# ducha-aiki/mods

Measured on AMD Instinct MI355X. Metric: image-pairs/sec (1024x768, HessAff+RootSIFT over the affine view ladder, MFMA FGINN match, LO-RANSAC H), higher is better.
Workload: dtype f32 (detect/describe) + u8 on the int8 matrix cores (distance matrix)

## Files before the change

include/modsx.h:

```cpp
#ifndef MODSX_H
#define MODSX_H
#include <stdint.h>
#ifdef __cplusplus
extern "C" {
#endif

#define MODSX_VERSION 100

typedef enum modsx_status {
  MODSX_OK = 0,
  MODSX_ERR_ARG = -1,
  MODSX_ERR_DEVICE = -2,
  MODSX_ERR_NOMEM = -3,
  MODSX_ERR_INTERNAL = -4,
  MODSX_ERR_CAPACITY = -5,
  MODSX_ERR_TIMEOUT = -6
} modsx_status;

enum { MODSX_FIXED_TH = 0, MODSX_RELATIVE_TH = 1, MODSX_FIXED_REG_NUMBER = 2, MODSX_RELATIVE_REG_NUMBER = 3,
       MODSX_NOT_LESS_THAN_REGIONS = 4 };
enum { MODSX_DET_HESSIAN = 0, MODSX_DET_DOG = 1, MODSX_DET_HARRIS = 2, MODSX_DET_MSER = 3 };
enum { MODSX_DESC_SIFT = 0, MODSX_DESC_ROOT_SIFT = 1, MODSX_DESC_HALF_SIFT = 2, MODSX_DESC_HALF_ROOT_SIFT = 3 };
#define MODSX_MAX_DESC 4
enum { MODSX_HESSIAN_DARK = 0, MODSX_HESSIAN_BRIGHT = 1, MODSX_HESSIAN_SADDLE = 2 };
// ... 166 lines not shown
int modsx_loransac_f(const double *pts, const double *laf1, const double *laf2, int T, double err_threshold,
                     double confidence, int max_samples, int localOptimization, double LAFCoef, int doSymmCheck,
                     int error_type, unsigned seed, double *F, unsigned char *inl, unsigned char *keep, int *data_out);
int modsx_verify_device_stats(long *out, int reset);
int modsx_verify_device_timing(long *out, int reset);

int modsx_match_pair(modsx_ctx *ctx, const modsx_image *img1, const modsx_image *img2,
                     const modsx_pair_params *par, modsx_pair_result *res);
void modsx_pair_result_release(modsx_pair_result *res);

int modsx_match_pairs(modsx_ctx *const *ctxs, int n_ctx, const modsx_image *const *imgs1,
                      const modsx_image *const *imgs2, int n_pairs, const modsx_pair_params *par,
                      modsx_pair_result *results);

int modsx_match_pairs_views(modsx_ctx *const *ctxs, int n_ctx, const modsx_image *const *imgs1,
                            const modsx_image *const *imgs2, int n_pairs, const modsx_view *views, int n_views,
                            const modsx_pair_params *par, modsx_pair_result *results);

int modsx_last_batch_verify(double *sum_ms, int *pairs, int *threads);
int modsx_last_match_geometry(int *qs, int *fat, int *S, int *tiles_per_split, int *ntiles_ub);
int modsx_debug_orientation_counts(unsigned long long *launched, unsigned long long *skipped, int reset);
int modsx_debug_reproject_certain_drop(const modsx_region *regs, int n, const double *H, int orig_w, int orig_h, double boxk,
                                       unsigned char *drop);
int modsx_last_timings(modsx_ctx *ctx, double *ms6);

int modsx_set_vs_pars(const double *scale_set, int ns, const double *tilt_set, int nt, double phi_base,
                      double InitSigma, int doBlur, modsx_view *par, int cap, modsx_view *prev, int *nprev,
                      int cap_prev);

modsx_image *modsx_synth_view(modsx_ctx *ctx, const modsx_image *gray, const modsx_view *view, double *H9,
                              int *is_identity);

int modsx_detect_describe_views(modsx_ctx *ctx, const modsx_image *img, const modsx_view *views, int nviews,
                                const modsx_pair_params *par, int view_begin, int view_step, modsx_region **regs,
                                float **desc, void *dev_desc_u8, long dev_cap, int *view_counts);

int modsx_match_fginn_device(modsx_ctx *ctx, const void *dev_desc1_u8, int n1, const void *dev_desc2_u8, int n2,
                             const double *pos2, double ratio, double contradDist, int nn, modsx_tentative **out);

#define MODSX_DB_MAX_ROWS 16777216L
typedef struct modsx_db modsx_db;
modsx_db *modsx_db_create(modsx_ctx *ctx, const void *rows, long n, int dtype);
void modsx_db_free(modsx_ctx *ctx, modsx_db *db);
long modsx_db_rows(const modsx_db *db);
int modsx_db_nearest(modsx_ctx *ctx, const modsx_db *db, const float *desc, int n, float *dmin);
int modsx_match_fginn_db(modsx_ctx *ctx, const float *desc1, int n1, const float *desc2, int n2, const double *pos2,
// ... 102 lines not shown
```

mods_amd/__init__.py:

```python
import ctypes as C
import os
import subprocess

import numpy as np

_HERE = os.path.dirname(os.path.abspath(__file__))
LIB_PATH = os.environ.get("MODSX_LIB", os.path.join(_HERE, "libmodsx.so"))

KEYPOINT = np.dtype([("x", "f8"), ("y", "f8"), ("a11", "f8"), ("a12", "f8"), ("a21", "f8"), ("a22", "f8"),
                     ("s", "f8"), ("response", "f8"), ("octave_number", "i4"), ("pyramid_scale", "f8"),
                     ("sub_type", "i4")], align=True)
REGION = np.dtype([("img_id", "i4"), ("img_reproj_id", "i4"), ("id", "i4"), ("parent_id", "i4"), ("type", "i4"),
                   ("det_kp", KEYPOINT), ("reproj_kp", KEYPOINT)], align=True)
SSKP = np.dtype([("octave", "i4"), ("level", "i4"), ("r0", "i4"), ("c0", "i4"), ("r", "i4"), ("c", "i4"),
                 ("type", "i4"), ("pad", "i4"), ("b0", "f4"), ("b1", "f4"), ("b2", "f4"), ("val", "f4"),
                 ("x", "f4"), ("y", "f4"), ("s", "f4"), ("pixelDistance", "f4")], align=True)
TENT = np.dtype([("q", "i4"), ("t0", "i4"), ("tj", "i4"), ("t1", "i4"), ("d1", "f8"), ("d2", "f8"),
                 ("d2by2ndcl", "f8"), ("ratio", "f8")], align=True)


class HessAffParams(C.Structure):
    _fields_ = [("threshold", C.c_float), ("mode", C.c_int), ("reg_number", C.c_int),
                ("rel_threshold", C.c_float), ("rel_reg_number", C.c_float), ("numberOfScales", C.c_int),
                ("initialSigma", C.c_float), ("edgeEigenValueRatio", C.c_double), ("border", C.c_int),
# ... 52 lines not shown


class RepClassSel(C.Structure):
    _fields_ = [("detector", C.c_int), ("desc_type", C.c_int), ("ratio", C.c_double)]


EXPORTS = ["modsx_version", "modsx_last_error", "modsx_free", "modsx_create", "modsx_destroy", "modsx_synchronize",
           "modsx_default_hessaff_params", "modsx_default_pair_params", "modsx_image_upload", "modsx_image_update",
           "modsx_image_wrap_device", "modsx_image_free", "modsx_image_download", "modsx_detect_affine_keypoints",
           "modsx_detect_scalespace", "modsx_octave_levels", "modsx_gaussian_blur", "modsx_resize_half", "modsx_response",
           "modsx_detect_affine_regions", "modsx_detect_orientation", "modsx_reproject_regions", "modsx_reproject_regions_touch_boundary",
           "modsx_describe_regions", "modsx_match_fginn", "modsx_duplicate_filtering", "modsx_ransac_h",
           "modsx_loransac_h", "modsx_ransac_h_errtype", "modsx_loransac_h_errtype", "modsx_ransac_f", "modsx_loransac_f", "modsx_match_pair", "modsx_match_pairs", "modsx_match_pairs_views", "modsx_pair_result_release",
           "modsx_set_vs_pars", "modsx_synth_view", "modsx_detect_describe_views", "modsx_match_fginn_device",
           "modsx_match_pair_views", "modsx_match_ladder", "modsx_save_regions", "modsx_load_regions", "modsx_default_mser_params", "modsx_detect_msers", "modsx_detect_msers_u8", "modsx_last_timings", "modsx_profile",
           "modsx_kernel_stats", "modsx_last_batch_verify", "modsx_last_match_geometry", "modsx_comm_unique_id", "modsx_comm_create", "modsx_comm_destroy", "modsx_comm_info",
           "modsx_view_block_order", "modsx_detect_describe_views_sharded", "modsx_match_fginn_sharded",
           "modsx_match_pair_views_sharded", "modsx_match_pairs_views_sharded", "modsx_match_ladder_sharded", "modsx_comm_loopback_id", "modsx_comm_set_lanes",
           "modsx_comm_attach", "modsx_comm_lane_done", "modsx_comm_reset_lanes", "modsx_comm_set_timeout", "modsx_comm_stats",
           "modsx_shard_block_bytes", "modsx_shard_block_pack", "modsx_shard_blocks_unpack", "modsx_shard_device_pack",
           "modsx_shard_device_unpack", "modsx_verify_device_stats", "modsx_verify_device_timing", "modsx_comm_set_exchange",
           "modsx_shard_owner_plan", "modsx_db_create", "modsx_db_free", "modsx_db_rows", "modsx_db_nearest",
           "modsx_match_fginn_db", "modsx_match_fginn_db_device", "modsx_set_fginn_db",
           "modsx_debug_orientation_counts", "modsx_debug_reproject_certain_drop",
           "modsx_rep_create", "modsx_rep_free", "modsx_rep_add_views", "modsx_rep_append", "modsx_rep_class",
           "modsx_rep_match_fginn", "modsx_match_reps", "modsx_match_one_to_many"]
EXPORTS_DEGENSAC = ["exp_ransacHcustom", "exp_ransacFcustom", "HDs", "HDsi", "HDsidx", "HDsSym", "HDsiSym", "HDsSymidx",
                    "HDsSymMax", "HDsiSymMax", "HDsSymidxMax", "FDs", "FDsSym", "exFDs", "exFDsSym",
                    "modsx_ransac_set_seed"]

SHARD_ROW_REGION, SHARD_ROW_KP = 0, 1
EXCHANGE_ALL_GATHER, EXCHANGE_OWNER = 0, 1
KP_FIELDS = ("x", "y", "a11", "a12", "a21", "a22", "s")
KERNEL_CLASSES = ["blur_hess", "hessian", "resize", "nms_localize", "baumberg", "orientation", "patch_sample",
                  "blur_rows", "describe", "match_fginn", "gray", "warp_affine", "view_blur", "blur_cols", "match_sweep1", "match_db"]


def build(force=False):
    src = os.path.join(_HERE, "csrc")
    srcs = [os.path.join(src, f) for f in os.listdir(src) if f.endswith((".hip", ".cpp", ".hpp"))]
    srcs.append(os.path.join(_HERE, "..", "include", "modsx.h"))
    stale = (not os.path.exists(LIB_PATH)) or any(os.path.getmtime(s) > os.path.getmtime(LIB_PATH) for s in srcs)
    if force or stale:
        subprocess.check_call(["make", "-C", src, "-j8"], stdout=subprocess.DEVNULL)
    return LIB_PATH


# ... 19 lines not shown
        L.modsx_comm_lane_done.argtypes = [C.c_void_p, C.c_int]
        L.modsx_comm_reset_lanes.argtypes = [C.c_void_p]
        L.modsx_comm_set_timeout.argtypes = [C.c_void_p, C.c_int]
        L.modsx_comm_stats.argtypes = [C.c_void_p, C.c_void_p, C.c_int]
        L.modsx_destroy.argtypes = [C.c_void_p]
        L.modsx_free.argtypes = [C.c_void_p]
        L.modsx_image_upload.restype = C.c_void_p
        L.modsx_image_upload.argtypes = [C.c_void_p, C.c_void_p, C.c_int, C.c_int, C.c_int, C.c_int]
        L.modsx_image_update.argtypes = [C.c_void_p, C.c_void_p, C.c_void_p, C.c_int, C.c_int, C.c_int, C.c_int]
        L.modsx_debug_last_batch_verify_each.argtypes = [C.c_void_p, C.c_int]
        L.modsx_image_wrap_device.restype = C.c_void_p
        L.modsx_image_wrap_device.argtypes = [C.c_void_p, C.c_void_p, C.c_int, C.c_int]
        L.modsx_image_free.argtypes = [C.c_void_p, C.c_void_p]
        L.modsx_db_create.restype = C.c_void_p
        L.modsx_db_create.argtypes = [C.c_void_p, C.c_void_p, C.c_long, C.c_int]
        L.modsx_db_free.restype = None
        L.modsx_db_free.argtypes = [C.c_void_p, C.c_void_p]
        L.modsx_db_rows.restype = C.c_long
        L.modsx_db_rows.argtypes = [C.c_void_p]
        L.modsx_db_nearest.argtypes = [C.c_void_p, C.c_void_p, C.c_void_p, C.c_int, C.c_void_p]
        L.modsx_set_fginn_db.argtypes = [C.c_void_p, C.c_void_p]
        L.modsx_debug_reproject_certain_drop.argtypes = [C.c_void_p, C.c_int, C.c_void_p, C.c_int, C.c_int, C.c_double, C.c_void_p]
        L.modsx_debug_orientation_counts.argtypes = [C.c_void_p, C.c_void_p, C.c_int]
        L.modsx_rep_create.restype = C.c_void_p
        L.modsx_rep_create.argtypes = [C.c_void_p]
        L.modsx_rep_free.restype = None
        L.modsx_rep_free.argtypes = [C.c_void_p, C.c_void_p]
        L.modsx_rep_add_views.argtypes = [C.c_void_p, C.c_void_p, C.c_void_p, C.c_void_p, C.c_void_p]
        L.modsx_rep_append.argtypes = [C.c_void_p, C.c_void_p, C.c_int, C.c_int, C.c_void_p, C.c_void_p, C.c_int, C.c_int]
        L.modsx_rep_class.argtypes = [C.c_void_p, C.c_void_p, C.c_int, C.c_int, C.c_void_p, C.c_void_p]
        L.modsx_rep_match_fginn.argtypes = [C.c_void_p, C.c_void_p, C.c_void_p, C.c_int, C.c_int, C.c_double, C.c_double, C.c_int,
                                            C.c_void_p]
        L.modsx_match_reps.argtypes = [C.c_void_p, C.c_int, C.c_void_p, C.c_void_p, C.c_int, C.c_void_p, C.c_int, C.c_void_p,
                                       C.c_void_p]
        L.modsx_match_one_to_many.argtypes = [C.c_void_p, C.c_int, C.c_void_p, C.c_void_p, C.c_int, C.c_void_p, C.c_int, C.c_int,
                                              C.c_void_p, C.c_void_p, C.c_void_p]
        L.modsx_synth_view.restype = C.c_void_p
        L.modsx_synth_view.argtypes = [C.c_void_p, C.c_void_p, C.c_void_p, C.c_void_p, C.c_void_p]
        _lib = L
    return _lib


def _err():
    return lib().modsx_last_error().decode()


# ... 616 lines not shown
    out = np.zeros(max(n, 1), np.float64)
    n = min(n, lib().modsx_debug_last_batch_verify_each(_p(out), len(out)))
    return out[:n]


def last_batch_verify():
    ms, n, t = C.c_double(), C.c_int(), C.c_int()
    lib().modsx_last_batch_verify(C.byref(ms), C.byref(n), C.byref(t))
    return ms.value, n.value, t.value


def last_match_geometry():
    v = [C.c_int() for _ in range(5)]
    lib().modsx_last_match_geometry(*[C.byref(x) for x in v])
    return dict(zip(("qs", "fat", "S", "tiles_per_split", "ntiles_ub"), (x.value for x in v)))


def orientation_counts(reset=False):
    a, b = C.c_ulonglong(), C.c_ulonglong()
    lib().modsx_debug_orientation_counts(C.byref(a), C.byref(b), int(reset))
    return a.value, b.value


def reproject_certain_drop(regs, H, w, h, boxk=2 * 3.0 * 3.0 ** 0.5):
    regs = np.ascontiguousarray(regs, REGION)
    H = np.ascontiguousarray(H, np.float64).reshape(9)
    drop = np.zeros(max(1, len(regs)), np.uint8)
    _check(lib().modsx_debug_reproject_certain_drop(_p(regs), len(regs), _p(H), int(w), int(h), C.c_double(boxk), _p(drop)),
           "reproject_certain_drop")
    return drop[:len(regs)].astype(bool)


def view_block_order(counts):
    counts = np.ascontiguousarray(counts, np.int32)
    world, nviews = counts.shape
    total = int(counts.sum())
    src = np.zeros(max(1, total), np.int32)
    mr = C.c_int(0)
    n = _check(lib().modsx_view_block_order(_p(counts), world, nviews, _p(src), len(src), C.byref(mr)), "view_block_order")
    return src[:n].copy(), mr.value


def shard_owner_plan(item_counts, nviews, world, rank, image_owner):
    cnt = np.ascontiguousarray(item_counts, np.int32)
    own = np.ascontiguousarray(image_owner, np.int32)
    nimg = len(own)
# ... 151 lines not shown
```

mods_amd/csrc/capi.hip:

```cpp
#include <math.h>
#include <malloc.h>
#include <atomic>
#include <chrono>
#include <mutex>
#include <thread>
#include <condition_variable>
#include <deque>
#include "engine_api.hpp"

using namespace mx;

#define NEED(c)                                             \
  do {                                                      \
    if (!(c)) { mx::set_error("null argument: " #c); return MODSX_ERR_ARG; } \
  } while (0)

template <typename T>
static T *to_malloc(const std::vector<T> &v) {
  T *p = (T *)malloc(sizeof(T) * (v.size() ? v.size() : 1));
  if (p && !v.empty()) memcpy(p, v.data(), sizeof(T) * v.size());
  return p;
}

static std::atomic<long> g_verifyUs(0);
// ... 303 lines not shown
  *out = to_malloc(vout[0]);
  return (int)vout[0].size();
}

int modsx_reproject_regions(modsx_region *regs, int n, const double *H, int orig_w, int orig_h) {
  if (n < 0 || (n > 0 && !regs) || !H) { mx::set_error("modsx_reproject_regions: bad argument"); return MODSX_ERR_ARG; }
  return reproject_regions(regs, n, H, orig_w, orig_h);
}

int modsx_reproject_regions_touch_boundary(modsx_region *regs, int n, const double *H, int orig_w, int orig_h, double mrSize) {
  if (n < 0 || (n > 0 && !regs) || !H) { mx::set_error("modsx_reproject_regions_touch_boundary: bad argument"); return MODSX_ERR_ARG; }
  return reproject_regions_box(regs, n, H, orig_w, orig_h, mrSize);
}

int modsx_debug_reproject_certain_drop(const modsx_region *regs, int n, const double *H, int orig_w, int orig_h, double boxk,
                                       unsigned char *drop) {
  if (n < 0 || (n > 0 && (!regs || !drop)) || !H) { mx::set_error("modsx_debug_reproject_certain_drop: bad argument"); return MODSX_ERR_ARG; }
  reproject_certain_drop(regs, n, H, orig_w, orig_h, boxk, drop);
  return n;
}

int modsx_debug_orientation_counts(unsigned long long *launched, unsigned long long *skipped, int reset) {
  mx::orientation_counts(launched, skipped, reset != 0);
  return MODSX_OK;
}

int modsx_describe_regions(modsx_ctx *ctx, const modsx_image *img, const modsx_region *regs, int n, double mrSize,
                           int patchSize, int fast_extraction, int photoNorm, int desc_type, double maxBinValue,
                           float *desc) {
  NEED(ctx); NEED(img);
  if (n < 0 || (n > 0 && (!regs || !desc))) { mx::set_error("modsx_describe_regions: bad argument"); return MODSX_ERR_ARG; }
  if (desc_type < MODSX_DESC_SIFT || desc_type > MODSX_DESC_HALF_ROOT_SIFT) { mx::set_error("descriptor type"); return MODSX_ERR_ARG; }
  hipSetDevice(ctx->dev);
  std::vector<modsx_region> v[1];
  v[0].assign(regs, regs + n);
  const modsx_image *imgs[1] = {img};
  float *hosts[1] = {desc};
  int rc = describe_batch(ctx, imgs, 1, v, mrSize, patchSize, fast_extraction, photoNorm, desc_type, maxBinValue, hosts,
                          nullptr, nullptr);
  if (rc) return rc;
  return n;
}

int modsx_match_fginn(modsx_ctx *ctx, const float *desc1, int n1, const float *desc2, int n2, const double *pos2,
                      double ratio, double contradDist, int nn, modsx_tentative **out) {
  NEED(ctx); NEED(out);
// ... 748 lines not shown
```

mods_amd/csrc/engine.hip:

```cpp
#include <atomic>
#include <math.h>
#include <stdio.h>
#include <algorithm>
#include <chrono>
#include <map>
#include <unordered_set>
#include <mutex>
#include <string>
#include "engine_api.hpp"

#ifdef MODSX_DUP_BUILD
namespace mx {
int dup_count(int cls) {
  static const long mask = getenv("MODSX_DUP") ? strtol(getenv("MODSX_DUP"), nullptr, 0) : 0;
  return 1 + (int)((mask >> cls) & 1);
}
}
#endif
namespace mx {

static thread_local std::string g_err;
void set_error(const std::string &s) { g_err = s; }
static std::atomic<int> g_busyContexts{0};
bool gpu_shared() { return g_busyContexts.load(std::memory_order_relaxed) > 1; }
// ... 175 lines not shown
  Profiler &p = c->prof;
  p.enabled = enable; p.used = 0;
  for (int i = 0; i < K_NCLASS; i++) { p.ms[i] = 0; p.work[i] = 0; p.launches[i] = 0; }
}

static int upload_tables(modsx_ctx *c) {
  const int PS = 41;
  std::vector<float> m(PS * PS);
  circular_gauss_mask(m.data(), PS, PS / 3.0f);
  {
    const int PSP = 44;
    std::vector<unsigned short> idx;
    std::vector<float> w;
    for (int r = 1; r < PS - 1; r++)
      for (int q = 1; q < PS - 1; q++)
        if (m[r * PS + q] > 0) { idx.push_back((unsigned short)(r * PSP + q)); w.push_back(m[r * PS + q]); }
    for (int r = 0; r < PS; r++)
      for (int q = 0; q < PS; q++)
        if ((r == 0 || q == 0 || r == PS - 1 || q == PS - 1) && m[r * PS + q] > 0) {
          set_error("orientation mask reaches the patch frame");
          return MODSX_ERR_ARG;
        }
    if ((int)idx.size() > ORI_NV) { set_error("orientation voting list exceeds ORI_NV"); return MODSX_ERR_ARG; }
    while ((int)idx.size() < ORI_NV) { idx.push_back((unsigned short)(PSP + 1)); w.push_back(0.f); }
    {
      constexpr int PER_L = ORI_NV / 64;
      std::vector<unsigned short> idx2(ORI_NV);
      std::vector<float> w2(ORI_NV);
      for (int l = 0; l < 64; l++)
        for (int q = 0; q < PER_L; q++) { idx2[l + 64 * q] = idx[PER_L * l + q]; w2[l + 64 * q] = w[PER_L * l + q]; }
      idx.swap(idx2); w.swap(w2);
    }
    MX_HIP(hipMalloc(&c->dOriMask, ORI_NV * 4));
    MX_HIP(hipMalloc(&c->dOriIdx, ORI_NV * 2));
    MX_HIP(hipMemcpy(c->dOriMask, w.data(), ORI_NV * 4, hipMemcpyHostToDevice));
    MX_HIP(hipMemcpy(c->dOriIdx, idx.data(), ORI_NV * 2, hipMemcpyHostToDevice));
  }
  MX_HIP(hipMalloc(&c->dSiftMask, PS * PS * 4));
  circular_gauss_mask(m.data(), PS, 0);
  MX_HIP(hipMemcpy(c->dSiftMask, m.data(), PS * PS * 4, hipMemcpyHostToDevice));
  {
    std::vector<unsigned short> idx;
    for (int i = 0; i < PS * PS; i++) if (m[i] > 0) idx.push_back((unsigned short)i);
    c->nSiftMask = (int)idx.size();
    MX_HIP(hipMalloc(&c->dSiftMaskIdx, idx.size() * 2));
    MX_HIP(hipMemcpy(c->dSiftMaskIdx, idx.data(), idx.size() * 2, hipMemcpyHostToDevice));
  }
  MX_HIP(hipMalloc(&c->dAtan, 256 * 8));
  MX_HIP(hipMemcpy(c->dAtan, atan_lut_host(), 256 * 8, hipMemcpyHostToDevice));
  {
    std::vector<unsigned char> obin(ATAN_CASES);
    std::vector<float> so(ATAN_CASES);
    const double *L = atan_lut_host();
    const float PIf = float(M_PI);
    const double TWO_PI = 6.28318530718;
    for (int e = 0; e < ATAN_CASES; e++) {
      const float ori = e < 2048 ? atan2lut_value(L, e >> 8, e & 255) : 0.f;
      obin[e] = (unsigned char)(int)(36 * (ori / PIf + 1.0f) / 2.0f);
      so[e] = (float)((double)8.0f * ((double)ori + TWO_PI) / TWO_PI);
// ... 60 lines not shown
  for (int i = 0; i < 6; i++) c->timings[i] = 0;
  if (upload_tables(c) != MODSX_OK) { delete c; return nullptr; }
  return c;
}

void ctx_destroy(modsx_ctx *c) {
  if (!c) return;
  ctx_worker_stop(c);
  if (c->peer) { ctx_destroy(c->peer); c->peer = nullptr; }
  if (c->half) { ctx_destroy(c->half); c->half = nullptr; }
  hipSetDevice(c->dev);
  hipStreamSynchronize(c->stream);
  for (int i = 0; i < MAXB; i++) c->pyr[i].store.release();
  DevBuf *bufs[] = {&c->nmsJobs, &c->cand, &c->counter, &c->affJobs, &c->affOut, &c->oriJobs, &c->oriOut, &c->descJobs, &c->tilePrefix,
                    &c->taps, &c->imgRefs, &c->scratchA, &c->scratchB, &c->descAllF[0], &c->descAllF[1], &c->descAllU8[0],
                    &c->descAllU8[1], &c->descAllU8b[0], &c->descAllU8b[1], &c->shardLocal, &c->pos2, &c->matchRows, &c->matchWork, &c->dbSel, &c->misc, &c->scratchC, &c->needTab, &c->coordTab, &c->tileJob, &c->blurTiles, &c->nmsQueue, &c->rowStarts, &c->viewTmp[0], &c->viewTmp[1], &c->viewTaps, &c->viewJobs};
  for (DevBuf *b : bufs) b->release();
  for (int i = 0; i < MAXB; i++) { c->descF[i].release(); c->descU8[i].release(); c->viewImg[i].release(); for (int k = 0; k < 3; k++) c->descU8x[k][i].release(); }
  for (int d = 0; d < 2; d++) for (int t = 0; t < 4; t++) for (int sd = 0; sd < 2; sd++) c->descCls[d][t][sd].release();
  for (int t = 0; t < 4; t++) c->halfDesc[t].release();
  c->candSort.release(); c->candOut.release();
  PinBuf *pins[] = {&c->hCand, &c->hAff, &c->hOri, &c->hDesc, &c->hMisc, &c->hNms, &c->hMatch, &c->hViewTaps, &c->hViewJobs, &c->hMser};
  for (PinBuf *b : pins) b->release();
  hipFree(c->dSmmMask); hipFree(c->dOriMask); hipFree(c->dOriIdx); hipFree(c->dSiftMask); hipFree(c->dSiftMaskIdx); hipFree(c->dAtan); hipFree(c->dOriBinTab); hipFree(c->dSiftOTab); hipFree(c->dSiftBins);
  hipFree(c->dSiftW);
  for (int i = 0; i < 2; i++) hipEventDestroy(c->descEv[i]);
  c->hDescB.release(); c->hRefs.release();
  hipStreamDestroy(c->stream);
  if (c->hFlag) hipHostFree(c->hFlag);
  delete c;
}

static const double K_SIGMA = 2 * 3.0 * sqrt(3.0);

void desc_class_order(const DescSet &ds, int *ord) {
  int m = 0;
  for (int type = 3; type >= 0; type--)
    for (int i = 0; i < ds.n; i++) if (ds.type[i] == type) ord[m++] = i;
}
int resolve_descs(const modsx_pair_params &pp, const modsx_ladder_step *st, DescSet &ds) {
  const int ns = st ? st->n_desc : 0;
  if (ns < 0 || ns > MODSX_MAX_DESC || pp.n_desc < 0 || pp.n_desc > MODSX_MAX_DESC) { set_error("n_desc must be 0..4"); return MODSX_ERR_ARG; }
  if (ns > 0) { ds.n = ns; for (int i = 0; i < ns; i++) { ds.type[i] = st->desc_types[i]; ds.ratio[i] = st->desc_ratios[i]; } }
  else if (pp.n_desc > 0) { ds.n = pp.n_desc; for (int i = 0; i < ds.n; i++) { ds.type[i] = pp.desc_types[i]; ds.ratio[i] = pp.desc_ratios[i]; } }
  else { ds.n = 1; ds.type[0] = pp.desc_type; ds.ratio[0] = st && st->match_ratio > 0 ? st->match_ratio : pp.match_ratio; }
  for (int i = 0; i < ds.n; i++) {
    if (ds.type[i] < 0 || ds.type[i] > 3) { set_error("descriptor type must be 0..3 (SIFT, RootSIFT, HalfSIFT, HalfRootSIFT)"); return MODSX_ERR_ARG; }
// ... 3 lines not shown
}

static int upload_img_refs(modsx_ctx *c, const modsx_image *const *imgs, int n) {
  const bool fresh = !c->imgRefs.p;
  if (!c->imgRefs.ensure(MAXB * sizeof(ImgRef))) return MODSX_ERR_NOMEM;
  ImgRef refs[MAXB];
  memset(refs, 0, sizeof refs);
  for (int i = 0; i < n; i++) { refs[i].d = imgs[i]->d; refs[i].rows = imgs[i]->rows; refs[i].cols = imgs[i]->cols; }
  if (!fresh && memcmp(refs, c->imgRefsHost, sizeof refs) == 0) return MODSX_OK;
  if (!c->hRefs.ensure(sizeof refs)) return MODSX_ERR_NOMEM;
  memcpy(c->hRefs.p, refs, sizeof refs);
  MX_HIP(ctx_copy(c, c->imgRefs.p, c->hRefs.p, sizeof refs, hipMemcpyHostToDevice));
  memcpy(c->imgRefsHost, refs, sizeof refs);
  return MODSX_OK;
}

static double eye_test(const double *H) {
  return fabs(H[0] - 1.0) + fabs(H[1]) + fabs(H[2]) + fabs(H[3]) + fabs(H[4] - 1.0) + fabs(H[5]) + fabs(H[6]) + fabs(H[7]) +
         fabs(H[8] - 1.0);
}
static bool is_eye(const double *H) { return eye_test(H) < 0.01; }
static bool ori_prefilter_on() {
  static const bool on = !(getenv("MODSX_ORI_PREFILTER") && atoi(getenv("MODSX_ORI_PREFILTER")) == 0);
  return on;
}
static std::atomic<unsigned long long> g_oriLaunched{0}, g_oriSkipped{0};
void orientation_counts(unsigned long long *launched, unsigned long long *skipped, bool reset) {
  if (launched) *launched = reset ? g_oriLaunched.exchange(0) : g_oriLaunched.load();
  else if (reset) g_oriLaunched.store(0);
  if (skipped) *skipped = reset ? g_oriSkipped.exchange(0) : g_oriSkipped.load();
  else if (reset) g_oriSkipped.store(0);
}

int detect_orientation_batch(modsx_ctx *c, const modsx_image *const *imgs, int n, const std::vector<modsx_region> *in,
                             double mrSize, int patchSize, int doHalfSIFT, int maxAngNum, double th, int addUpRight,
                             std::vector<modsx_region> *out, const OriReproj *reproj) {
  if (patchSize != 41) { set_error("orientation patchSize must be 41"); return MODSX_ERR_ARG; }
  const bool prefilter = reproj && ori_prefilter_on();
  for (int i = 0; i < n; i++) out[i].clear();
  double mrScale = (double)mrSize;
  int patchImageSize = 2 * int(mrScale) + 1;
  double imageToPatchScale = double(patchImageSize) / (double)patchSize;
  HostMark hm;
  std::vector<OriJob> jobs;
  std::vector<char> passed[MAXB];
  std::vector<unsigned char> certain[MAXB];
// ... 30 lines not shown
  jobStart[0] = 0;
  for (int i = 0; i < n; i++) jobStart[i + 1] = jobStart[i] + jobsOf[i].size();
  jobs.resize(jobStart[n]);
  g_oriLaunched.fetch_add(jobStart[n], std::memory_order_relaxed);
  host_parallel_light(n, [&](int i) { if (!jobsOf[i].empty()) memcpy(jobs.data() + jobStart[i], jobsOf[i].data(), jobsOf[i].size() * sizeof(OriJob)); });
  hm.mark("orientation jobs");
  const float *res = nullptr;
  const int maxA = maxAngNum < 0 ? ORI_MAX_PEAKS : std::min(maxAngNum, ORI_MAX_PEAKS);
  const size_t oriB = (size_t)(1 + maxA) * 4;
  if (!jobs.empty()) {
    int rc = upload_img_refs(c, imgs, n);
    if (rc) return rc;
    hipStream_t s = c->stream;
    size_t nj = jobs.size();
    if (!c->oriJobs.ensure(nj * sizeof(OriJob)) || !c->oriOut.ensure(nj * oriB) ||
        !c->hOri.ensure(nj * (sizeof(OriJob) + oriB)))
      return MODSX_ERR_NOMEM;
    memcpy(c->hOri.p, jobs.data(), nj * sizeof(OriJob));
    float *hres = (float *)((char *)c->hOri.p + nj * sizeof(OriJob));
    res = hres;
    MX_HIP(ctx_copy(c, c->oriJobs.p, c->hOri.p, nj * sizeof(OriJob), hipMemcpyHostToDevice));
    ProfScope ps(c, K_ORIENT, (double)nj * 41 * 41 * 4);
    launch_orientation(s, (OriJob *)c->oriJobs.p, (float *)c->oriOut.p, (int)nj, (ImgRef *)c->imgRefs.p, c->dOriIdx,
                       c->dOriMask, c->dOriBinTab, doHalfSIFT, th, maxA);
    MX_HIP(ctx_copy(c, hres, c->oriOut.p, nj * oriB, hipMemcpyDeviceToHost));
    MX_HIP(ctx_sync(c));
  }
  hm.mark("orientation launch + wait");
  host_parallel_light(n, [&](int i) {
    size_t jk = jobStart[i];
    out[i].clear();
    out[i].reserve(in[i].size() + in[i].size() / 4);
    for (size_t r = 0; r < in[i].size(); r++) {
      if (!passed[i][r]) continue;
      const modsx_region &base = in[i][r];
      if (maxAngNum > 0) {
        const float *o = res + (jk++) * (size_t)(1 + maxA);
        int on;
        memcpy(&on, o, 4);
        const double b11 = base.det_kp.a11, b12 = base.det_kp.a12, b21 = base.det_kp.a21, b22 = base.det_kp.a22;
        for (int a = 0; a < on; a++) {
          double ci = cosf(-o[1 + a]);
          double si = sinf(-o[1 + a]);
          out[i].push_back(base);
          modsx_region &t = out[i].back();
          t.id = 0;
          t.det_kp.a11 = b11 * ci - b12 * si;
// ... 809 lines not shown
```

mods_amd/csrc/engine.hpp:

```cpp
#pragma once
#include <hip/hip_runtime.h>
#include <stdint.h>
#include <stdlib.h>
#include <string.h>
#include <string>
#include <vector>
#include "../../include/modsx.h"
#include "kmath.hpp"

namespace mx {

#ifndef MODSX_MAXB
#define MODSX_MAXB 32
#endif
constexpr int MAXB = MODSX_MAXB;
constexpr int PAIR_GROUP = 4;
constexpr int NMS_MAXJ = 1024;
constexpr int MAX_TAPS = 17;

struct BlurJob {
  const float *src;
  float *blur;
  float *resp;
  int rows, cols;
// ... 153 lines not shown
inline bool check_borders_host(int w, int h, float ofsx, float ofsy, float a11, float a12, float a21, float a22, int rw, int rh) {
  return check_borders(w, h, ofsx, ofsy, a11, a12, a21, a22, rw, rh);
}
bool invert3(const double *S, double *t);
void rectify(double &a11, double &a12, double &a21, double &a22);

void launch_blur_hess(hipStream_t s, const BlurBatch &b, int nj, int maxRows, int maxCols);
void launch_hessian(hipStream_t s, const BlurBatch &b, int nj, int maxRows, int maxCols);
void launch_resize_half(hipStream_t s, const ResizeBatch &b, int nj, int maxRows, int maxCols);
void launch_nms(hipStream_t s, const NmsBatch &b, const NmsJob *jobs, const int *tilePrefix, const int *tileJob, int nj,
                int nTiles, int4 *queue, unsigned *qcount, unsigned qcap, Candidate *out, unsigned *counter, unsigned cap,
                const int *octFirst = nullptr, int levelsPerOctave = 0);
size_t cand_sort_temp_bytes(unsigned nsort);
int launch_cand_order(hipStream_t s, const Candidate *cand, const unsigned *counter, unsigned nsort, unsigned long long *keys,
                      unsigned long long *keys2, unsigned *idx, unsigned *idx2, void *temp, size_t tempBytes, unsigned long long *tabKey,
                      unsigned *tabRank, unsigned tabSize, unsigned *slotOf, Candidate *out, unsigned *outCount);
constexpr int NMS_QUEUES = 64;
constexpr int NMS_TILE_ROWS = 16;
void launch_gray(hipStream_t s, const void *src, float *dst, size_t n, int channels, int dtype);
void launch_baumberg(hipStream_t s, const AffJob *jobs, AffOut *out, int n, const float *mask, int W, int maxIter,
                     float convTh, float affInitialSigma);
constexpr int ATAN_CASES = 2048 + 64;
constexpr int ORI_NV = 1344;
void launch_orientation(hipStream_t s, const OriJob *jobs, float *out, int n, const ImgRef *imgs,
                        const unsigned short *maskIdx, const float *maskW,
                        const unsigned char *binTab, int doHalf, double th, int maxAngles);
void launch_trunc_u8(hipStream_t s, const float *src, uint8_t *dst, size_t n);
size_t mser_sort_blocks(const int *rows, int n);
void launch_mser_sort(hipStream_t s, const uint8_t *const *u8, const int *rows, const int *cols, const size_t *ordOfs, int n, int *blockHist,
                      int *start, int *order);
void launch_expand_blur_tiles(hipStream_t s, const DescJob *jobs, const int *prefixRows, const int *prefixCols, int nJobs,
                              const int *needTab, BlurTile *tilesRows, BlurTile *tilesCols, float2 *rowStarts);
void launch_sample_rows(hipStream_t s, const DescJob *jobs, const BlurTile *tiles, int nTiles, const ImgRef *imgs, const float *taps,
                        const int *needTab, float *dst, const float2 *rowStarts, float *dstGrid);
void launch_blur_cols(hipStream_t s, const BlurTile *tiles, int nTiles, const float *taps, const int *needTab, const float *src,
                      float *dst);
void launch_expand_tiles(hipStream_t s, const int *prefix, int nJobs, int *tileJob);
void launch_patch_sample(hipStream_t s, const DescJob *jobs, const int *tilePrefix, const int *tileJob, int nTiles,
                         const ImgRef *imgs, float *scratch);
void launch_patch_blur(hipStream_t s, const DescJob *jobs, const int *tilePrefix, const int *tileJob, int nTiles,
                       const float *taps, const int *needTab, const float *src, float *dst, int pass);
void launch_describe(hipStream_t s, const DescJob *jobs, int n, const ImgRef *imgs, const float *grid,
                     const int *needTab, const float *coordTab,
                     const float *mask, const unsigned short *maskIdx, int nmask, const float *oTab, const int *bins,
                     const double *wts, int photoNorm, int descTypes, int nOut, double maxBin, const DescOut &outs);
void launch_warp_affine(hipStream_t s, const WarpJob &jb);
void launch_blur_pass(hipStream_t s, const float *src, float *dst, int rows, int cols, const float *taps, int n, int pass, int border = 0);
void launch_sub(hipStream_t s, const float *a, const float *b, float *o, size_t n);
// ... 83 lines not shown
  size_t lastSurvivors = 0;
  mx::DevBuf nmsJobs, cand, counter, affJobs, affOut, oriJobs, oriOut, descJobs, tilePrefix, taps, imgRefs, scratchA, scratchB,
      descF[mx::MAXB], descU8[mx::MAXB], descAllF[2], descAllU8[2], descAllU8b[2], descCls[2][4][2], descU8x[3][mx::MAXB], shardLocal, pos2, matchRows, matchWork, dbSel, misc, viewTmp[2], viewTaps, viewJobs, viewImg[mx::MAXB], scratchC, needTab, coordTab, tileJob, blurTiles, nmsQueue, rowStarts;
  mx::ImgRef imgRefsHost[mx::MAXB];
  mx::PinBuf hDescB;
  hipEvent_t descEv[2];
  bool descEvPending[2] = {false, false};
  bool descByEvent[2] = {true, true};
  unsigned descMark[2] = {0, 0};
  unsigned *hFlag = nullptr;
  unsigned flagSeq = 0;
  bool waitRuntime = true;
  mx::PinBuf hCand, hAff, hOri, hDesc, hMisc, hNms, hMatch, hViewTaps, hViewJobs, hMser, hRefs;
  float *dSmmMask = nullptr;
  int smmW = 0;
  std::vector<uint64_t> candKeys, candKeys2, candClaim;
  std::vector<uint32_t> candOrder, candOrder2;
  float *dOriMask = nullptr;
  unsigned short *dOriIdx = nullptr;
  float *dSiftMask = nullptr;
  unsigned short *dSiftMaskIdx = nullptr;
  int nSiftMask = 0;
  double *dAtan = nullptr;
  unsigned char *dOriBinTab = nullptr;
  float *dSiftOTab = nullptr;
  int *dSiftBins = nullptr;
  double *dSiftW = nullptr;
  double timings[6];
  mx::Profiler prof;
  size_t lastCandCount = 0;
  const mx::DbSet *fginnDb = nullptr;
  int busyDepth = 0;
  int shardLane = 0;
  modsx_ctx *peer = nullptr;
  modsx_ctx *half = nullptr;
  mx::DevBuf halfDesc[4];
  void *worker = nullptr;
};
```

mods_amd/csrc/kernels_orient.hip:

```cpp
#include "engine.hpp"

namespace mx {

constexpr int PS = 41, PSP = 44;
constexpr int ORI_B = 21;

template <bool LDS_TABLE>
__global__ __launch_bounds__(64) void k_orientation(const OriJob *jobs, float *out, int n, const ImgRef *imgs,
                                                    const unsigned short *maskIdx, const float *maskW,
                                                    const unsigned char *binTab, int doHalf, double th, int maxAngles) {
  const int k = xcd_chunk(blockIdx.x, n);
  if (k >= n) return;
  const int lane = threadIdx.x;
  __shared__ __attribute__((aligned(16))) float bufX[PS * PSP];
  __shared__ __attribute__((aligned(16))) unsigned char sbtLds[LDS_TABLE ? ATAN_CASES : 16];
  const unsigned char *const sbt = LDS_TABLE ? sbtLds : binTab;
  __shared__ float hist[40];
  static_assert(ATAN_CASES == 33 * 64, "one 4-byte word per lane and step");
  if (LDS_TABLE) {
    unsigned t[9];
#pragma unroll
    for (int u = 0; u < 9; u++) t[u] = lane + 64 * u < ATAN_CASES / 4 ? reinterpret_cast<const unsigned *>(binTab)[lane + 64 * u] : 0u;
#pragma unroll
    for (int u = 0; u < 9; u++)
      if (lane + 64 * u < ATAN_CASES / 4) reinterpret_cast<unsigned *>(sbtLds)[lane + 64 * u] = t[u];
  }
  const OriJob jb = jobs[k];
  const ImgRef im = imgs[jb.img];
  const int half = PS >> 1;
  const bool touch = check_borders(im.cols, im.rows, jb.x, jb.y, jb.a11, jb.a12, jb.a21, jb.a22, PS, PS);
  {
    float rx = jb.x - (float)half * jb.a12, ry = jb.y - (float)half * jb.a22;
#pragma unroll
    for (int j = 1; j < PS; j++)
      if (lane >= j) { rx += jb.a12; ry += jb.a22; }
    if (lane < PS) {
      float WX = rx - (float)half * jb.a11;
      float WY = ry - (float)half * jb.a21;
      float *row = bufX + lane * PSP;
      for (int i0 = 0; i0 < PS; i0 += ORI_B) {
        float t[ORI_B];
        if (!touch) {
#pragma unroll
          for (int u = 0; u < ORI_B; u++) {
            t[u] = i0 + u < PS ? bilinear_tap(as_global(im.d), im.rows, im.cols, WX, WY, false) : 0.f;
            WX += jb.a11; WY += jb.a21;
          }
        } else {
#pragma unroll
          for (int u = 0; u < ORI_B; u++) {
            t[u] = i0 + u < PS ? bilinear_tap(as_global(im.d), im.rows, im.cols, WX, WY, true) : 0.f;
            WX += jb.a11; WY += jb.a21;
          }
        }
#pragma unroll
        for (int u = 0; u < ORI_B; u++)
          if (i0 + u < PS) row[i0 + u] = t[u];
      }
    }
  }
  __syncthreads();
  const float PIf = float(M_PI);
  constexpr int PER_L = ORI_NV / 64;
  float wreg[PER_L];
  unsigned char breg[PER_L];
#pragma unroll
  for (int q = 0; q < PER_L; q++) {
    const int e = lane + 64 * q;
    const int p = maskIdx[e];
    const float m = maskW[e];
    const float xg = bufX[p + 1] - bufX[p - 1];
    const float yg = bufX[p + PSP] - bufX[p - PSP];
    const float mag = sqrtf(xg * xg + yg * yg);
    int code, idx;
    const bool special = atan2lut_case(yg, xg, code, idx);
    unsigned char bin = 255;
    float w = 0.f;
    if (m > 0 && mag > 1.0f) {
      bin = sbt[special ? 2048 : code * 256 + idx];
      w = mag * m;
// ... 84 lines not shown
  float mx = lane < nb ? hv : 0.f;
#pragma unroll
  for (int off = 32; off > 0; off >>= 1) mx = fmaxf(mx, __shfl_xor(mx, off));
  const float thresh = (float)((double)(mx > 0.f ? mx : 0.f) * th);
  if (doHalf) {
    const float other = __shfl(hv, lane < nb / 2 ? lane + nb / 2 : lane);
    if (lane < nb / 2) hv += other;
    else if (lane < nb) hv = 0.f;
  }
  const float ha = __shfl(hv, lane == 0 ? nb - 1 : lane - 1);
  const float hc = __shfl(hv, lane == nb - 1 ? 0 : lane + 1);
  const bool peak = lane < nb && hv >= thresh && hv > ha && hv > hc;
  const unsigned long long peaks = __ballot(peak);
  const int rank = __popcll(peaks & ((1ull << lane) - 1ull));
  float *const o = out + (size_t)k * (1 + maxAngles);
  if (lane == 0) o[0] = __int_as_float(min(__popcll(peaks), maxAngles));
  if (peak && rank < maxAngles) {
    const float pp = (ha - hc) / (ha - 2.0f * hv + hc) / 2.0f;
    o[1 + rank] = 2.0f * PIf * ((float)lane + 0.5f + pp) / (float)nb - PIf;
  }
}

void launch_orientation(hipStream_t s, const OriJob *jobs, float *out, int n, const ImgRef *imgs,
                          const unsigned short *maskIdx, const float *maskW, const unsigned char *binTab, int doHalf, double th,
                          int maxAngles) {
  if (n <= 0) return;
  if (n < 2 * 256 * 16)
    MX_DUP(K_ORIENT) hipLaunchKernelGGL(k_orientation<true>, dim3(8 * ((n + 7) / 8)), dim3(64), 0, s, jobs, out, n, imgs, maskIdx, maskW, binTab, doHalf, th,
                       maxAngles);
  else
    MX_DUP(K_ORIENT) hipLaunchKernelGGL(k_orientation<false>, dim3(8 * ((n + 7) / 8)), dim3(64), 0, s, jobs, out, n, imgs, maskIdx, maskW, binTab, doHalf, th,
                       maxAngles);
}

}
```

mods_amd/csrc/tables.cpp:

```cpp
#include <math.h>
#include <stdio.h>
#include "engine.hpp"

namespace mx {

std::vector<float> gaussian_kernel(int n, double sigma) {
  std::vector<float> k(n);
  double sigmaX = sigma > 0 ? sigma : ((n - 1) * 0.5 - 1) * 0.3 + 0.8;
  double scale2X = -0.5 / (sigmaX * sigmaX);
  double sum = 0;
  for (int i = 0; i < n; i++) {
    double x = i - (n - 1) * 0.5;
    double t = exp(scale2X * x * x);
    k[i] = (float)t;
    sum += k[i];
  }
  sum = 1. / sum;
  for (int i = 0; i < n; i++) k[i] = (float)(k[i] * sum);
  return k;
}

int blur_ksize(float sigma) {
  int size = (int)(2.0 * 3.0 * sigma + 1.0);
  if (size % 2 == 0) size++;
// ... 9 lines not shown
  int endSize = int(ceilf(scale * 5.0f) - halfSize);
  for (int i = 1; i < endSize; i++) tmp[halfSize - i] += expf(float((i + halfSize) * (i + halfSize)) / scale2);
  for (int i = 0; i <= halfSize; i++)
    for (int j = 0; j <= halfSize; j++) {
      float v = tmp[i] * tmp[j];
      mask[(i + halfSize) * size + (-j + halfSize)] = v;
      mask[(-i + halfSize) * size + (j + halfSize)] = v;
      mask[(i + halfSize) * size + (j + halfSize)] = v;
      mask[(-i + halfSize) * size + (-j + halfSize)] = v;
    }
}

void circular_gauss_mask(float *mask, int size, float sigma) {
  int halfSize = size >> 1;
  float r2 = float(halfSize * halfSize);
  float sigma2 = (sigma == 0) ? 0.9f * r2 : 2 * sigma * sigma;
  for (int i = 0; i < size; i++)
    for (int j = 0; j < size; j++) {
      float disq = float((i - halfSize) * (i - halfSize) + (j - halfSize) * (j - halfSize));
      mask[i * size + j] = (disq < r2) ? expf(-disq / sigma2) : 0;
    }
}

const double *atan_lut_host() {
  static double lut[256];
  static bool ready = false;
  if (!ready) {
    for (int i = 0; i < 256; i++) {
      char buf[64];
      snprintf(buf, sizeof buf, "%.10f", atan(i / 255.0));
      lut[i] = strtod(buf, nullptr);
    }
    lut[32] = 0.1248376255;
    lut[83] = 0.3146752558;
    lut[100] = 0.3737268255;
    ready = true;
  }
  return lut;
}

bool invert3(const double *S, double *t) {
  double d = S[0] * (S[4] * S[8] - S[5] * S[7]) - S[1] * (S[3] * S[8] - S[5] * S[6]) + S[2] * (S[3] * S[7] - S[4] * S[6]);
  if (d == 0.) { for (int i = 0; i < 9; i++) t[i] = 0; return false; }
  d = 1. / d;
  t[0] = (S[4] * S[8] - S[5] * S[7]) * d; t[1] = (S[2] * S[7] - S[1] * S[8]) * d; t[2] = (S[1] * S[5] - S[2] * S[4]) * d;
  t[3] = (S[5] * S[6] - S[3] * S[8]) * d; t[4] = (S[0] * S[8] - S[2] * S[6]) * d; t[5] = (S[2] * S[3] - S[0] * S[5]) * d;
// ... 16 lines not shown
```

Measured before the change: 221.9.

## Sample only voting-relevant orientation patch taps, spread evenly across all 64 lanes

The orientation kernel used to have lanes 0..40 each sample a full 41-pixel patch row while the other lanes sat idle. It now precomputes, on the host, the set of pixels whose value feeds a masked gradient vote. That set is the circular mask dilated by one pixel in each direction. It is split into per-lane runs of at most 22 taps, each covering up to two row segments, and packed into a small device table. The kernel reads its lane's run and bilinearly samples only those taps, which drops corner samples and uses the whole wavefront. The trade-offs are extra per-lane address setup, padding voting entries redirected to the patch centre, and a new env toggle plus a debug export.

```diff
diff --git a/include/modsx.h b/include/modsx.h
--- a/include/modsx.h
+++ b/include/modsx.h
@@ -212,6 +212,7 @@
 int modsx_debug_orientation_counts(unsigned long long *launched, unsigned long long *skipped, int reset);
 int modsx_debug_reproject_certain_drop(const modsx_region *regs, int n, const double *H, int orig_w, int orig_h, double boxk,
                                        unsigned char *drop);
+int modsx_debug_orientation_tap_shares(int *share, int *needed, int *max_len);
 int modsx_last_timings(modsx_ctx *ctx, double *ms6);
 
 int modsx_set_vs_pars(const double *scale_set, int ns, const double *tilt_set, int nt, double phi_base,
diff --git a/mods_amd/__init__.py b/mods_amd/__init__.py
--- a/mods_amd/__init__.py
+++ b/mods_amd/__init__.py
@@ -98,7 +98,7 @@
            "modsx_shard_device_unpack", "modsx_verify_device_stats", "modsx_verify_device_timing", "modsx_comm_set_exchange",
            "modsx_shard_owner_plan", "modsx_db_create", "modsx_db_free", "modsx_db_rows", "modsx_db_nearest",
            "modsx_match_fginn_db", "modsx_match_fginn_db_device", "modsx_set_fginn_db",
-           "modsx_debug_orientation_counts", "modsx_debug_reproject_certain_drop",
+           "modsx_debug_orientation_counts", "modsx_debug_reproject_certain_drop", "modsx_debug_orientation_tap_shares",
            "modsx_rep_create", "modsx_rep_free", "modsx_rep_add_views", "modsx_rep_append", "modsx_rep_class",
            "modsx_rep_match_fginn", "modsx_match_reps", "modsx_match_one_to_many"]
 EXPORTS_DEGENSAC = ["exp_ransacHcustom", "exp_ransacFcustom", "HDs", "HDsi", "HDsidx", "HDsSym", "HDsiSym", "HDsSymidx",
@@ -164,6 +164,7 @@
         L.modsx_set_fginn_db.argtypes = [C.c_void_p, C.c_void_p]
         L.modsx_debug_reproject_certain_drop.argtypes = [C.c_void_p, C.c_int, C.c_void_p, C.c_int, C.c_int, C.c_double, C.c_void_p]
         L.modsx_debug_orientation_counts.argtypes = [C.c_void_p, C.c_void_p, C.c_int]
+        L.modsx_debug_orientation_tap_shares.argtypes = [C.c_void_p, C.c_void_p, C.c_void_p]
         L.modsx_rep_create.restype = C.c_void_p
         L.modsx_rep_create.argtypes = [C.c_void_p]
         L.modsx_rep_free.restype = None
@@ -826,6 +827,13 @@
     return a.value, b.value
 
 
+def orientation_tap_shares():
+    share = np.zeros((64, 5), np.int32)
+    a, b = C.c_int(), C.c_int()
+    _check(lib().modsx_debug_orientation_tap_shares(_p(share), C.byref(a), C.byref(b)), "orientation_tap_shares")
+    return share, a.value, b.value
+
+
 def reproject_certain_drop(regs, H, w, h, boxk=2 * 3.0 * 3.0 ** 0.5):
     regs = np.ascontiguousarray(regs, REGION)
     H = np.ascontiguousarray(H, np.float64).reshape(9)
diff --git a/mods_amd/csrc/capi.hip b/mods_amd/csrc/capi.hip
--- a/mods_amd/csrc/capi.hip
+++ b/mods_amd/csrc/capi.hip
@@ -349,6 +349,16 @@
 
 int modsx_debug_orientation_counts(unsigned long long *launched, unsigned long long *skipped, int reset) {
   mx::orientation_counts(launched, skipped, reset != 0);
+  return MODSX_OK;
+}
+
+int modsx_debug_orientation_tap_shares(int *share, int *needed, int *max_len) {
+  if (!share) { mx::set_error("modsx_debug_orientation_tap_shares: bad argument"); return MODSX_ERR_ARG; }
+  std::vector<float> m(41 * 41);
+  mx::circular_gauss_mask(m.data(), 41, 41 / 3.0f);
+  mx::OriTapShare s[64];
+  if (!mx::orientation_tap_shares(m.data(), s, needed, max_len)) { mx::set_error("orientation tap shares do not fit ORI_TAP_LEN"); return MODSX_ERR_ARG; }
+  for (int l = 0; l < 64; l++) { share[5 * l] = s[l].row; share[5 * l + 1] = s[l].c0; share[5 * l + 2] = s[l].len0; share[5 * l + 3] = s[l].c1; share[5 * l + 4] = s[l].len1; }
   return MODSX_OK;
 }
 
diff --git a/mods_amd/csrc/engine.hip b/mods_amd/csrc/engine.hip
--- a/mods_amd/csrc/engine.hip
+++ b/mods_amd/csrc/engine.hip
@@ -221,7 +221,7 @@
           return MODSX_ERR_ARG;
         }
     if ((int)idx.size() > ORI_NV) { set_error("orientation voting list exceeds ORI_NV"); return MODSX_ERR_ARG; }
-    while ((int)idx.size() < ORI_NV) { idx.push_back((unsigned short)(PSP + 1)); w.push_back(0.f); }
+    while ((int)idx.size() < ORI_NV) { idx.push_back((unsigned short)((PS / 2) * PSP + PS / 2)); w.push_back(0.f); }
     {
       constexpr int PER_L = ORI_NV / 64;
       std::vector<unsigned short> idx2(ORI_NV);
@@ -234,6 +234,12 @@
     MX_HIP(hipMalloc(&c->dOriIdx, ORI_NV * 2));
     MX_HIP(hipMemcpy(c->dOriMask, w.data(), ORI_NV * 4, hipMemcpyHostToDevice));
     MX_HIP(hipMemcpy(c->dOriIdx, idx.data(), ORI_NV * 2, hipMemcpyHostToDevice));
+    OriTapShare share[64];
+    unsigned packed[64];
+    if (!orientation_tap_shares(m.data(), share, nullptr, nullptr)) { set_error("orientation tap shares do not fit ORI_TAP_LEN"); return MODSX_ERR_ARG; }
+    for (int l = 0; l < 64; l++) packed[l] = ori_tap_pack(share[l]);
+    MX_HIP(hipMalloc(&c->dOriTaps, sizeof packed));
+    MX_HIP(hipMemcpy(c->dOriTaps, packed, sizeof packed, hipMemcpyHostToDevice));
   }
   MX_HIP(hipMalloc(&c->dSiftMask, PS * PS * 4));
   circular_gauss_mask(m.data(), PS, 0);
@@ -340,7 +346,7 @@
   c->candSort.release(); c->candOut.release();
   PinBuf *pins[] = {&c->hCand, &c->hAff, &c->hOri, &c->hDesc, &c->hMisc, &c->hNms, &c->hMatch, &c->hViewTaps, &c->hViewJobs, &c->hMser};
   for (PinBuf *b : pins) b->release();
-  hipFree(c->dSmmMask); hipFree(c->dOriMask); hipFree(c->dOriIdx); hipFree(c->dSiftMask); hipFree(c->dSiftMaskIdx); hipFree(c->dAtan); hipFree(c->dOriBinTab); hipFree(c->dSiftOTab); hipFree(c->dSiftBins);
+  hipFree(c->dSmmMask); hipFree(c->dOriMask); hipFree(c->dOriIdx); hipFree(c->dOriTaps);hipFree(c->dSiftMask); hipFree(c->dSiftMaskIdx); hipFree(c->dAtan); hipFree(c->dOriBinTab); hipFree(c->dSiftOTab); hipFree(c->dSiftBins);
   hipFree(c->dSiftW);
   for (int i = 0; i < 2; i++) hipEventDestroy(c->descEv[i]);
   c->hDescB.release(); c->hRefs.release();
@@ -390,6 +396,10 @@
 static bool is_eye(const double *H) { return eye_test(H) < 0.01; }
 static bool ori_prefilter_on() {
   static const bool on = !(getenv("MODSX_ORI_PREFILTER") && atoi(getenv("MODSX_ORI_PREFILTER")) == 0);
+  return on;
+}
+static bool ori_flat_taps_on() {
+  static const bool on = !(getenv("MODSX_ORI_FLAT_TAPS") && atoi(getenv("MODSX_ORI_FLAT_TAPS")) == 0);
   return on;
 }
 static std::atomic<unsigned long long> g_oriLaunched{0}, g_oriSkipped{0};
@@ -466,7 +476,7 @@
     MX_HIP(ctx_copy(c, c->oriJobs.p, c->hOri.p, nj * sizeof(OriJob), hipMemcpyHostToDevice));
     ProfScope ps(c, K_ORIENT, (double)nj * 41 * 41 * 4);
     launch_orientation(s, (OriJob *)c->oriJobs.p, (float *)c->oriOut.p, (int)nj, (ImgRef *)c->imgRefs.p, c->dOriIdx,
-                       c->dOriMask, c->dOriBinTab, doHalfSIFT, th, maxA);
+                       c->dOriMask, ori_flat_taps_on() ? c->dOriTaps : nullptr, c->dOriBinTab, doHalfSIFT, th, maxA);
     MX_HIP(ctx_copy(c, hres, c->oriOut.p, nj * oriB, hipMemcpyDeviceToHost));
     MX_HIP(ctx_sync(c));
   }
diff --git a/mods_amd/csrc/engine.hpp b/mods_amd/csrc/engine.hpp
--- a/mods_amd/csrc/engine.hpp
+++ b/mods_amd/csrc/engine.hpp
@@ -199,8 +199,14 @@
                      float convTh, float affInitialSigma);
 constexpr int ATAN_CASES = 2048 + 64;
 constexpr int ORI_NV = 1344;
+constexpr int ORI_TAP_LEN = 22, ORI_TAP_C1MAX = 14;
+struct OriTapShare { int row, c0, len0, c1, len1; };
+bool orientation_tap_shares(const float *mask, OriTapShare *share64, int *nNeeded, int *maxLen);
+inline unsigned ori_tap_pack(const OriTapShare &s) {
+  return (unsigned)s.row | (unsigned)s.c0 << 6 | (unsigned)s.len0 << 12 | (unsigned)s.c1 << 17 | (unsigned)(s.len0 + s.len1) << 23;
+}
 void launch_orientation(hipStream_t s, const OriJob *jobs, float *out, int n, const ImgRef *imgs,
-                        const unsigned short *maskIdx, const float *maskW,
+                        const unsigned short *maskIdx, const float *maskW, const unsigned *tapShares,
                         const unsigned char *binTab, int doHalf, double th, int maxAngles);
 void launch_trunc_u8(hipStream_t s, const float *src, uint8_t *dst, size_t n);
 size_t mser_sort_blocks(const int *rows, int n);
@@ -330,6 +336,7 @@
   unsigned short *dSiftMaskIdx = nullptr;
   int nSiftMask = 0;
   double *dAtan = nullptr;
+  unsigned *dOriTaps = nullptr;
   unsigned char *dOriBinTab = nullptr;
   float *dSiftOTab = nullptr;
   int *dSiftBins = nullptr;
diff --git a/mods_amd/csrc/kernels_orient.hip b/mods_amd/csrc/kernels_orient.hip
--- a/mods_amd/csrc/kernels_orient.hip
+++ b/mods_amd/csrc/kernels_orient.hip
@@ -5,9 +5,9 @@
 constexpr int PS = 41, PSP = 44;
 constexpr int ORI_B = 21;
 
-template <bool LDS_TABLE>
+template <bool LDS_TABLE, bool FLAT>
 __global__ __launch_bounds__(64) void k_orientation(const OriJob *jobs, float *out, int n, const ImgRef *imgs,
-                                                    const unsigned short *maskIdx, const float *maskW,
+                                                    const unsigned short *maskIdx, const float *maskW, const unsigned *tapShares,
                                                     const unsigned char *binTab, int doHalf, double th, int maxAngles) {
   const int k = xcd_chunk(blockIdx.x, n);
   if (k >= n) return;
@@ -29,33 +29,71 @@
   const ImgRef im = imgs[jb.img];
   const int half = PS >> 1;
   const bool touch = check_borders(im.cols, im.rows, jb.x, jb.y, jb.a11, jb.a12, jb.a21, jb.a22, PS, PS);
-  {
+  if (FLAT) {
+    const unsigned sg = tapShares[lane];
+    const int srow = sg & 63, c0 = (sg >> 6) & 63, n0 = (sg >> 12) & 31, c1 = (sg >> 17) & 63, nt = (sg >> 23) & 31;
     float rx = jb.x - (float)half * jb.a12, ry = jb.y - (float)half * jb.a22;
 #pragma unroll
     for (int j = 1; j < PS; j++)
-      if (lane >= j) { rx += jb.a12; ry += jb.a22; }
-    if (lane < PS) {
-      float WX = rx - (float)half * jb.a11;
-      float WY = ry - (float)half * jb.a21;
-      float *row = bufX + lane * PSP;
-      for (int i0 = 0; i0 < PS; i0 += ORI_B) {
-        float t[ORI_B];
-        if (!touch) {
-#pragma unroll
-          for (int u = 0; u < ORI_B; u++) {
-            t[u] = i0 + u < PS ? bilinear_tap(as_global(im.d), im.rows, im.cols, WX, WY, false) : 0.f;
-            WX += jb.a11; WY += jb.a21;
+      if (srow >= j) { rx += jb.a12; ry += jb.a22; }
+    float WX = rx - (float)half * jb.a11, WY = ry - (float)half * jb.a21;
+    rx += jb.a12; ry += jb.a22;
+    float VX = rx - (float)half * jb.a11, VY = ry - (float)half * jb.a21;
+#pragma unroll
+    for (int j = 1; j < PS; j++)
+      if (c0 >= j) { WX += jb.a11; WY += jb.a21; }
+#pragma unroll
+    for (int j = 1; j <= ORI_TAP_C1MAX; j++)
+      if (c1 >= j) { VX += jb.a11; VY += jb.a21; }
+    float *const run0 = bufX + srow * PSP + c0, *const run1 = bufX + (srow + 1) * PSP + c1 - n0;
+    float t[ORI_TAP_LEN];
+    if (!touch) {
+#pragma unroll
+      for (int u = 0; u < ORI_TAP_LEN; u++) {
+        if (u == n0) { WX = VX; WY = VY; }
+        t[u] = bilinear_tap(as_global(im.d), im.rows, im.cols, WX, WY, false);
+        WX += jb.a11; WY += jb.a21;
+      }
+    } else {
+#pragma unroll
+      for (int u = 0; u < ORI_TAP_LEN; u++) {
+        if (u == n0) { WX = VX; WY = VY; }
+        t[u] = bilinear_tap(as_global(im.d), im.rows, im.cols, WX, WY, true);
+        WX += jb.a11; WY += jb.a21;
+      }
+    }
+#pragma unroll
+    for (int u = 0; u < ORI_TAP_LEN; u++)
+      if (u < nt) (u < n0 ? run0 : run1)[u] = t[u];
+  } else {
+    {
+      float rx = jb.x - (float)half * jb.a12, ry = jb.y - (float)half * jb.a22;
+  #pragma unroll
+      for (int j = 1; j < PS; j++)
+        if (lane >= j) { rx += jb.a12; ry += jb.a22; }
+      if (lane < PS) {
+        float WX = rx - (float)half * jb.a11;
+        float WY = ry - (float)half * jb.a21;
+        float *row = bufX + lane * PSP;
+        for (int i0 = 0; i0 < PS; i0 += ORI_B) {
+          float t[ORI_B];
+          if (!touch) {
+  #pragma unroll
+            for (int u = 0; u < ORI_B; u++) {
+              t[u] = i0 + u < PS ? bilinear_tap(as_global(im.d), im.rows, im.cols, WX, WY, false) : 0.f;
+              WX += jb.a11; WY += jb.a21;
+            }
+          } else {
+  #pragma unroll
+            for (int u = 0; u < ORI_B; u++) {
+              t[u] = i0 + u < PS ? bilinear_tap(as_global(im.d), im.rows, im.cols, WX, WY, true) : 0.f;
+              WX += jb.a11; WY += jb.a21;
+            }
           }
-        } else {
-#pragma unroll
-          for (int u = 0; u < ORI_B; u++) {
-            t[u] = i0 + u < PS ? bilinear_tap(as_global(im.d), im.rows, im.cols, WX, WY, true) : 0.f;
-            WX += jb.a11; WY += jb.a21;
-          }
+  #pragma unroll
+          for (int u = 0; u < ORI_B; u++)
+            if (i0 + u < PS) row[i0 + u] = t[u];
         }
-#pragma unroll
-        for (int u = 0; u < ORI_B; u++)
-          if (i0 + u < PS) row[i0 + u] = t[u];
       }
     }
   }
@@ -186,15 +224,19 @@
 }
 
 void launch_orientation(hipStream_t s, const OriJob *jobs, float *out, int n, const ImgRef *imgs,
-                          const unsigned short *maskIdx, const float *maskW, const unsigned char *binTab, int doHalf, double th,
-                          int maxAngles) {
+                          const unsigned short *maskIdx, const float *maskW, const unsigned *tapShares, const unsigned char *binTab,
+                          int doHalf, double th, int maxAngles) {
   if (n <= 0) return;
-  if (n < 2 * 256 * 16)
-    MX_DUP(K_ORIENT) hipLaunchKernelGGL(k_orientation<true>, dim3(8 * ((n + 7) / 8)), dim3(64), 0, s, jobs, out, n, imgs, maskIdx, maskW, binTab, doHalf, th,
-                       maxAngles);
-  else
-    MX_DUP(K_ORIENT) hipLaunchKernelGGL(k_orientation<false>, dim3(8 * ((n + 7) / 8)), dim3(64), 0, s, jobs, out, n, imgs, maskIdx, maskW, binTab, doHalf, th,
-                       maxAngles);
+  const dim3 grid(8 * ((n + 7) / 8));
+  const bool small = n < 2 * 256 * 16;
+#define MX_ORI_LAUNCH(LT, FL) \
+  MX_DUP(K_ORIENT) hipLaunchKernelGGL((k_orientation<LT, FL>), grid, dim3(64), 0, s, jobs, out, n, imgs, maskIdx, maskW, tapShares, binTab, doHalf, th, maxAngles)
+  if (tapShares) {
+    if (small) MX_ORI_LAUNCH(true, true); else MX_ORI_LAUNCH(false, true);
+  } else {
+    if (small) MX_ORI_LAUNCH(true, false); else MX_ORI_LAUNCH(false, false);
+  }
+#undef MX_ORI_LAUNCH
 }
 
 }
diff --git a/mods_amd/csrc/tables.cpp b/mods_amd/csrc/tables.cpp
--- a/mods_amd/csrc/tables.cpp
+++ b/mods_amd/csrc/tables.cpp
@@ -55,6 +55,52 @@
     }
 }
 
+bool orientation_tap_shares(const float *mask, OriTapShare *share64, int *nNeeded, int *maxLen) {
+  const int PS = 41;
+  int first[PS], count[PS], total = 0;
+  for (int r = 0; r < PS; r++) {
+    first[r] = -1; count[r] = 0;
+    int last = -1;
+    for (int q = 0; q < PS; q++) {
+      auto votes = [&](int rr, int qq) { return rr >= 0 && qq >= 0 && rr < PS && qq < PS && mask[rr * PS + qq] > 0; };
+      if (votes(r, q) || votes(r - 1, q) || votes(r + 1, q) || votes(r, q - 1) || votes(r, q + 1)) {
+        if (first[r] < 0) first[r] = q;
+        last = q; count[r]++;
+      }
+    }
+    if (count[r] == 0 || last - first[r] + 1 != count[r]) return false;
+    total += count[r];
+  }
+  const int cap = (total + 63) / 64;
+  if (cap > ORI_TAP_LEN) return false;
+  int r = 0, q = first[0], longest = 0;
+  for (int l = 0; l < 64; l++) {
+    OriTapShare s = {0, 0, 0, 0, 0};
+    if (r < PS) {
+      s.row = r; s.c0 = q;
+      s.len0 = std::min(cap, first[r] + count[r] - q);
+      q += s.len0;
+      if (q == first[r] + count[r]) {
+        r++;
+        q = r < PS ? first[r] : 0;
+        if (r < PS && s.len0 < cap) {
+          s.c1 = q;
+          s.len1 = std::min(cap - s.len0, count[r]);
+          q += s.len1;
+          if (s.len1 == count[r]) { r++; q = r < PS ? first[r] : 0; }
+        }
+      }
+    }
+    if (s.c1 > ORI_TAP_C1MAX) return false;
+    longest = std::max(longest, s.len0 + s.len1);
+    share64[l] = s;
+  }
+  if (r < PS) return false;
+  if (nNeeded) *nNeeded = total;
+  if (maxLen) *maxLen = longest;
+  return true;
+}
+
 const double *atan_lut_host() {
   static double lut[256];
   static bool ready = false;
```

Measured after the change: 223.6, median of 6. Within noise of the previous version (+0.7%).
